# eragonruan/text-detection-ctpn

Measured on NVIDIA H100. Metric: images/sec @600x900, higher is better.
Workload: dtype fp32-faithful: fp16 operands + e4m3 cross terms (1 fp16 + 1 e4m3 wgmma per 16 MACs: 2 bf16-rate units per MAC), fp32 accumulate; matmuls around the BiLSTM on bf16x2

## Files before the change

text-detection-ctpn_b200/csrc/conv_tc.cu:

```cuda
#include <cuda.h>

#include <algorithm>
#include <mutex>
#include <unordered_map>

#include "common.cuh"
#include "tc_ptx.cuh"
#include "tma_host.cuh"

namespace ctpn {

#ifdef CTPN_DEBUG
#define CTPN_DBG(p, bit) (((p).debug & (bit)) != 0)
#else
#define CTPN_DBG(p, bit) false
#endif

struct ConvTcParams {
  int B, H, W, Cin, Cout, taps, planes, flags;
  int tiles_x, tiles_y, tiles_n, total_tiles;
  int m_tiles, total_units;
  int TH, TW, tw_log2;
  int PW;
  int patch_bytes;
  int patch_tx_bytes;
  int group_stride_bytes;
  int cout_pad;
  int Ho, Wo;
  int stages_a, stages_b;
  int debug;
  const float *bias;
  void *out;
  long long out_plane_stride;
  float inv_main, inv_cross, out_s, out_t, out_rs;
  int in_stack_h, out_rows, out_stacked;
  const int *ext;
  int ext_shift, ext_n;
  double work;
  int promote_every;
};

template <int BN, int PR> constexpr bool kEpiWarpgroup = !PR && BN <= 128;
template <int BN, int PR> constexpr int kTcThreads = kEpiWarpgroup<BN, PR> ? 512 : 384;
constexpr int kMaxStages = 8;
constexpr int kCtrlBytes = 8 * (4 * kMaxStages) + 16;
constexpr int kEpiBytes = 2 * 128 * 32 * 4;
constexpr int kXposeBytes = 4 * 512;

struct EpiPixel {
  bool ok, live;
  int oy, ox;
  long long pix;
  unsigned okmask;
  long long spix[4];
};

__device__ __forceinline__ void epi_pixel(const ConvTcParams &p, int mt, int m, int lane, EpiPixel &e) {
  const int th = m >> p.tw_log2, tw = m & (p.TW - 1);
  const int tiles_per_img = p.tiles_x * p.tiles_y;
  const int b = mt / tiles_per_img, r = mt % tiles_per_img;
  const int y = (r / p.tiles_x) * p.TH + th, x = (r % p.tiles_x) * p.TW + tw;
  e.live = true;
  int ob = b;
  if (p.flags & CTPN_F_POOL) {
    e.oy = y >> 1; e.ox = x >> 1;
    e.ok = !(th & 1) && !(tw & 1) && e.oy < p.Ho && e.ox < p.Wo;
  } else {
    e.oy = y; e.ox = x;
    e.ok = y < p.H && x < p.W;
    if (p.in_stack_h) {
      ob = y / p.in_stack_h;
      e.oy = y - ob * p.in_stack_h;
      e.live = e.oy < p.in_stack_h - 1;
      if (!p.out_stacked) e.ok = e.ok && e.live;
    }
  }
  if (p.ext) {
    const int ib = min(ob, p.ext_n - 1);
    e.live = e.live && e.oy < (__ldg(p.ext + 2 * ib) >> p.ext_shift) && e.ox < (__ldg(p.ext + 2 * ib + 1) >> p.ext_shift);
  }
  e.pix = ((long long)ob * p.out_rows + e.oy) * p.Wo + e.ox;
  e.okmask = __ballot_sync(0xffffffffu, e.ok);
#pragma unroll
  for (int it = 0; it < 4; ++it) {
    const long long hi = __shfl_sync(0xffffffffu, (int)(e.pix >> 32), it * 8 + (lane >> 2));
    const unsigned lo = __shfl_sync(0xffffffffu, (unsigned)(e.pix & 0xffffffffll), it * 8 + (lane >> 2));
    e.spix[it] = (hi << 32) | lo;
  }
}

__device__ __forceinline__ void store_transposed(uint4 *stage_w, const uint32_t (&w)[16], uint8_t *obase, long long row_bytes,
                                                 const EpiPixel &e, bool st_ok, bool small, int lane) {
  const int j = lane & 3;
  if (!small) {
    __syncwarp();
#pragma unroll
    for (int q = 0; q < 4; ++q) stage_w[lane * 4 + (q ^ ((lane >> 1) & 3))] = make_uint4(w[4 * q], w[4 * q + 1], w[4 * q + 2], w[4 * q + 3]);
    __syncwarp();
    if (st_ok) {
#pragma unroll
      for (int it = 0; it < 4; ++it) {
        const int pp = it * 8 + (lane >> 2);
        const uint4 val = stage_w[pp * 4 + (j ^ ((pp >> 1) & 3))];
        if ((e.okmask >> pp) & 1u) *reinterpret_cast<uint4 *>(obase + e.spix[it] * row_bytes) = val;
      }
    }
  } else {
#pragma unroll
    for (int it = 0; it < 4; ++it) {
      __syncwarp();
      if ((lane >> 3) == it) {
        const int row = lane & 7;
#pragma unroll
        for (int q = 0; q < 4; ++q) stage_w[row * 4 + (q ^ ((row >> 1) & 3))] = make_uint4(w[4 * q], w[4 * q + 1], w[4 * q + 2], w[4 * q + 3]);
      }
      __syncwarp();
      const int row = lane >> 2, pp = it * 8 + row;
      const uint4 val = stage_w[row * 4 + (j ^ ((row >> 1) & 3))];
      if (st_ok && ((e.okmask >> pp) & 1u)) *reinterpret_cast<uint4 *>(obase + e.spix[it] * row_bytes) = val;
    }
  }
}

template <int P, int F8>
__device__ __forceinline__ void epi_chunk(const ConvTcParams &p, const EpiPixel &e, float (&v)[32], int c0, uint4 *stage_w,
                                          bool small, bool bias_relu, int lane) {
  const bool pool = (p.flags & CTPN_F_POOL) != 0, relu = (p.flags & CTPN_F_RELU) != 0;
  const bool out_f32 = (p.flags & CTPN_F_OUT_F32) != 0;
  if (bias_relu) {
#pragma unroll
    for (int q = 0; q < 8; ++q) {
      const float4 bq = __ldg(reinterpret_cast<const float4 *>(p.bias + c0) + q);
      v[4 * q + 0] += bq.x;
      v[4 * q + 1] += bq.y;
      v[4 * q + 2] += bq.z;
      v[4 * q + 3] += bq.w;
    }
    if (relu) {
#pragma unroll
      for (int i = 0; i < 32; ++i) v[i] = fmaxf(v[i], 0.f);
    }
  }
  if (!e.live) {
#pragma unroll
    for (int i = 0; i < 32; ++i) v[i] = 0.f;
  }
  if (pool) {
#pragma unroll
    for (int i = 0; i < 32; ++i) {
      v[i] = fmaxf(v[i], __shfl_xor_sync(0xffffffffu, v[i], 1));
      v[i] = fmaxf(v[i], __shfl_xor_sync(0xffffffffu, v[i], p.TW));
    }
  }
  if (F8 && pool && !out_f32 && !(p.flags & CTPN_F_OUT_BF16X2)) {
    const int j = (lane & 1) | ((lane >> 2) & 2);
    float x[8];
#pragma unroll
    for (int k = 0; k < 8; ++k) x[k] = j == 0 ? v[k] : j == 1 ? v[8 + k] : j == 2 ? v[16 + k] : v[24 + k];
    const bool okw = e.oy < p.Ho && e.ox < p.Wo;
    uint4 hw;
    uint2 qv, qr;
    f16f8_quad(x[0], x[1], x[2], x[3], p.out_s, p.out_t, p.out_rs, hw.x, hw.y, qv.x, qr.x);
    f16f8_quad(x[4], x[5], x[6], x[7], p.out_s, p.out_t, p.out_rs, hw.z, hw.w, qv.y, qr.y);
    if (okw && c0 < p.Cout && !CTPN_DBG(p, 8)) {
      uint8_t *o0 = reinterpret_cast<uint8_t *>(p.out) + e.pix * p.Cout * 2;
      uint8_t *o1 = o0 + p.out_plane_stride * 2 + (long long)(c0 >> 6) * 128 + (c0 & 63) + j * 8;
      *reinterpret_cast<uint4 *>(o0 + (long long)c0 * 2 + j * 16) = hw;
      *reinterpret_cast<uint2 *>(o1) = qv;
      *reinterpret_cast<uint2 *>(o1 + 64) = qr;
    }
  } else if (F8 && !out_f32 && !(p.flags & CTPN_F_OUT_BF16X2)) {
    uint32_t wh[16], wq[16];
#pragma unroll
    for (int i = 0; i < 8; ++i) {
      f16f8_quad(v[4 * i], v[4 * i + 1], v[4 * i + 2], v[4 * i + 3], p.out_s, p.out_t, p.out_rs, wh[2 * i], wh[2 * i + 1], wq[i], wq[8 + i]);
    }
    const int j = lane & 3;
    const bool st_ok = c0 < p.Cout && !CTPN_DBG(p, 8);
    uint8_t *obase = reinterpret_cast<uint8_t *>(p.out);
    store_transposed(stage_w, wh, obase + (long long)c0 * 2 + j * 16, (long long)p.Cout * 2, e, st_ok, small, lane);
    store_transposed(stage_w, wq, obase + p.out_plane_stride * 2 + (long long)(c0 >> 6) * 128 + (c0 & 63) + (j >> 1) * 64 + (j & 1) * 16,
                     (long long)p.Cout * 2, e, st_ok, small, lane);
  } else if (!out_f32) {
    uint32_t w[P][16];
#pragma unroll
    for (int i = 0; i < 16; ++i) {
      uint32_t t[P];
      split_planes2<P>(v[2 * i], v[2 * i + 1], t);
#pragma unroll
      for (int pl = 0; pl < P; ++pl) w[pl][i] = t[pl];
    }
#pragma unroll
    for (int pl = 0; pl < P; ++pl) {
      uint8_t *obase = reinterpret_cast<uint8_t *>(reinterpret_cast<__nv_bfloat16 *>(p.out) + (long long)pl * p.out_plane_stride + c0 + (lane & 3) * 8);
      store_transposed(stage_w, w[pl], obase, (long long)p.Cout * 2, e, c0 < p.Cout && !CTPN_DBG(p, 8), small, lane);
    }
  } else if (e.ok && c0 < p.Cout && !CTPN_DBG(p, 8)) {
    float4 *dst = reinterpret_cast<float4 *>(reinterpret_cast<float *>(p.out) + e.pix * p.Cout + c0);
#pragma unroll
    for (int q = 0; q < 8; ++q) dst[q] = make_float4(v[4 * q], v[4 * q + 1], v[4 * q + 2], v[4 * q + 3]);
  }
}

template <int BN, int P, int TAPS, int MC, int F8, int PR = 0>
__global__ void __launch_bounds__(kTcThreads<BN, PR>, 1)
conv_tc_kernel(const __grid_constant__ CUtensorMap tmap_a, const __grid_constant__ CUtensorMap tmap_b,
               const ConvTcParams p) {
  using namespace ptx;
  constexpr int kBBytes = BN * 128;
  constexpr bool EW = kEpiWarpgroup<BN, PR>;
  static_assert(!F8 || P == 2, "F16F8 uses two stage slots per operand");
  static_assert(!PR || (P == 3 && !F8), "promotion is built for three bf16 planes");
  extern __shared__ uint8_t smem_raw[];
  const uint32_t raw = smem_u32(smem_raw);
  const uint32_t ring_a = (raw + 1023u) & ~1023u;
  const uint32_t a_stage = (uint32_t)P * p.patch_bytes, b_stage = (uint32_t)P * kBBytes;
  const uint32_t ring_b = ring_a + (uint32_t)p.stages_a * a_stage;
  float *epi = reinterpret_cast<float *>(smem_raw + (ring_b - raw) + (size_t)p.stages_b * b_stage);
  uint4 *xpose = reinterpret_cast<uint4 *>(reinterpret_cast<uint8_t *>(epi) + kEpiBytes);
  uint8_t *ctrl = reinterpret_cast<uint8_t *>(epi) + kEpiBytes + (EW ? kXposeBytes : 0);
  const uint32_t fullA = smem_u32(ctrl), emptyA = fullA + 8 * kMaxStages;
  const uint32_t fullB = emptyA + 8 * kMaxStages, emptyB = fullB + 8 * kMaxStages;
  const uint32_t epiF = emptyB + 8 * kMaxStages, epiE = epiF + 8;

  const int warp = __shfl_sync(0xffffffffu, (int)(threadIdx.x >> 5), 0), lane = threadIdx.x & 31;
  if (threadIdx.x == 0) {
    prefetch_tmap(&tmap_a);
    prefetch_tmap(&tmap_b);
    for (int s = 0; s < kMaxStages; ++s) {
      mbar_init(fullA + 8 * s, 1);
      mbar_init(emptyA + 8 * s, 2);
      mbar_init(fullB + 8 * s, 1);
      mbar_init(emptyB + 8 * s, MC ? 4 : 2);
    }
    mbar_init(epiF, 256);
    mbar_init(epiE, 128);
    fence_mbar_init();
  }
  __syncthreads();
  if (MC) cluster_sync_all();
  const uint32_t rank = MC ? cluster_ctarank() : 0u;
  const int u_begin = MC ? (int)(blockIdx.x >> 1) : (int)blockIdx.x, u_step = MC ? (int)(gridDim.x >> 1) : (int)gridDim.x;
  auto unit_tile = [&](int u, int &mt, int &nt) {
    nt = u % p.tiles_n;
    mt = u / p.tiles_n;
    if (MC) mt = min(2 * mt + (int)rank, p.m_tiles - 1);
  };

  const int kblocks = p.Cin / 64;
  const int tiles_per_img = p.tiles_x * p.tiles_y;
  constexpr int halo = TAPS == 9 ? 1 : 0;

  if (warp < 4) {
    if (EW) regs_dealloc<24>();
    else regs_dealloc<40>();
    if (warp == 1) {
      int s = 0;
      uint32_t ph = 0;
      for (int u = u_begin; u < p.total_units; u += u_step) {
        int mt, nt;
        unit_tile(u, mt, nt);
        const int b = mt / tiles_per_img, r = mt % tiles_per_img;
        const int y0 = (r / p.tiles_x) * p.TH - halo, x0 = (r % p.tiles_x) * p.TW - halo;
        for (int kb = 0; kb < kblocks; ++kb) {
          mbar_wait(emptyA + 8 * s, ph ^ 1u);
          if (elect_one()) {
            if (CTPN_DBG(p, 2)) { mbar_arrive(fullA + 8 * s); }
            else {
              mbar_arrive_expect_tx(fullA + 8 * s, (uint32_t)P * (uint32_t)p.patch_tx_bytes);
              for (int pl = 0; pl < P; ++pl)
                tma_load_4d(&tmap_a, fullA + 8 * s, ring_a + s * a_stage + pl * p.patch_bytes, kb * 64, x0, y0, pl * p.B + b);
            }
          }
          __syncwarp();
          if (++s == p.stages_a) { s = 0; ph ^= 1u; }
        }
      }
    } else if (warp == 0) {
      int s = 0;
      uint32_t ph = 0;
      for (int u = u_begin; u < p.total_units; u += u_step) {
        int mt, nt;
        unit_tile(u, mt, nt);
        for (int kb = 0; kb < kblocks; ++kb) {
          for (int tap = 0; tap < TAPS; ++tap) {
            mbar_wait(emptyB + 8 * s, ph ^ 1u);
            if (elect_one()) {
              if (CTPN_DBG(p, 1)) { mbar_arrive(fullB + 8 * s); }
              else {
                mbar_arrive_expect_tx(fullB + 8 * s, b_stage);
                for (int pl = 0; pl < P; ++pl) {
                  if (MC)
                    tma_load_2d_mc(&tmap_b, fullB + 8 * s, ring_b + s * b_stage + pl * kBBytes + rank * (kBBytes / 2),
                                   tap * p.Cin + kb * 64, pl * p.cout_pad + nt * BN + (int)rank * (BN / 2), (uint16_t)3);
                  else
                    tma_load_2d(&tmap_b, fullB + 8 * s, ring_b + s * b_stage + pl * kBBytes, tap * p.Cin + kb * 64,
                                pl * p.cout_pad + nt * BN);
                }
              }
            }
            __syncwarp();
            if (++s == p.stages_b) { s = 0; ph ^= 1u; }
          }
        }
      }
    }
  } else if (EW && warp >= 12) {
    regs_alloc<152>();
    const int m = (warp & 3) * 32 + lane;
    uint4 *stage_w = xpose + (warp & 3) * 32;
    uint32_t eph = 0;
    if (!CTPN_DBG(p, 16)) {
      for (int u = u_begin; u < p.total_units; u += u_step) {
        int mt, nt;
        unit_tile(u, mt, nt);
        EpiPixel e;
        epi_pixel(p, mt, m, lane, e);
#pragma unroll 1
        for (int c2 = 0; c2 < BN / 64; ++c2) {
          float v[2][32];
          mbar_wait(epiF, eph);
#pragma unroll
          for (int es = 0; es < 2; ++es) {
#pragma unroll
            for (int q = 0; q < 8; ++q) {
              const float4 t = *reinterpret_cast<const float4 *>(epi + es * 4096 + m * 32 + ((q ^ (m & 7)) << 2));
              v[es][4 * q + 0] = t.x; v[es][4 * q + 1] = t.y; v[es][4 * q + 2] = t.z; v[es][4 * q + 3] = t.w;
            }
          }
          mbar_arrive(epiE);
          eph ^= 1u;
#pragma unroll
          for (int es = 0; es < 2; ++es) epi_chunk<P, F8>(p, e, v[es], nt * BN + (2 * c2 + es) * 32, stage_w, true, false, lane);
        }
      }
    }
  } else {
    if (EW) regs_alloc<168>();
    else regs_alloc<232>();
    const int wg = (warp >> 2) - 1;
    const bool leader = (threadIdx.x & 127) == 0;
    constexpr int R = BN / 2;
    float accm[R], accc[R];
    float accs[R];
#ifdef CTPN_DEBUG
    const int pe = PR ? p.promote_every : 1;
#else
    constexpr int pe = 1;
#endif
    constexpr uint32_t kPatch16 = (TAPS == 9 ? 23552u : 16384u) >> 4;
    constexpr uint32_t kB16 = (uint32_t)kBBytes >> 4;
    constexpr uint32_t kHiB = gmma_desc_hi(1024);
    const uint32_t hi_a = gmma_desc_hi((uint32_t)p.group_stride_bytes);
    const uint32_t wg_off = (uint32_t)wg * 8u * (uint32_t)p.group_stride_bytes;
    int sa = 0, sb = 0, prev_b = -1, prev_a = -1;
    uint32_t pha = 0, phb = 0, eph = 0;
    const int frow = wg * 64 + (warp & 3) * 16 + (lane >> 2);
    auto stage_half = [&](int c2) {
#pragma unroll
      for (int j = 0; j < 8; ++j) {
        const int i8 = c2 * 8 + j, q = 2 * (j & 3) + ((lane & 3) >> 1);
#pragma unroll
        for (int h = 0; h < 2; ++h) {
          const int row = frow + 8 * h;
          *reinterpret_cast<float2 *>(epi + (j >> 2) * 4096 + row * 32 + ((q ^ (row & 7)) << 2) + 2 * (lane & 1)) =
              make_float2(accm[4 * i8 + 2 * h], accm[4 * i8 + 2 * h + 1]);
        }
      }
    };
    auto release = [&](int sbx, int sax) {
      if (leader) {
        if (MC) {
          mbar_arrive_cluster(emptyB + 8 * sbx, 0u);
          mbar_arrive_cluster(emptyB + 8 * sbx, 1u);
        } else {
          mbar_arrive(emptyB + 8 * sbx);
        }
        if (sax >= 0) mbar_arrive(emptyA + 8 * sax);
      }
    };
    for (int u = u_begin; u < p.total_units; u += u_step) {
      if (PR) {
#pragma unroll
        for (int i = 0; i < R; ++i) accs[i] = 0.f;
      }
      for (int kb = 0; kb < kblocks; ++kb) {
        if (p.stages_a == 1 && prev_a >= 0) {
          wgmma_wait<0>();
          release(prev_b, prev_a);
          prev_b = prev_a = -1;
        }
        mbar_wait(fullA + 8 * sa, pha);
        const uint32_t a_lo = gmma_desc_lo(ring_a + sa * a_stage + wg_off);
#pragma unroll
        for (int tap = 0; tap < TAPS; ++tap) {
          mbar_wait(fullB + 8 * sb, phb);
          const uint32_t b_lo = gmma_desc_lo(ring_b + sb * b_stage);
          constexpr int kPW = 10;
          const uint32_t view16 = TAPS == 9 ? (uint32_t)((tap / 3) * kPW + tap % 3) * 8u : 0u;
          const uint32_t not_first = (kb | tap) != 0;
          const int step = kb * TAPS + tap;
          wgmma_fence();
          if (!CTPN_DBG(p, 4)) {
            if (F8) {
#pragma unroll
              for (int k = 0; k < 4; ++k)
                wgmma_f16(accm, ((uint64_t)hi_a << 32) | (a_lo + view16 + 2u * k), ((uint64_t)kHiB << 32) | (b_lo + 2u * k),
                          k == 0 ? not_first : 1u);
#pragma unroll
              for (int k = 0; k < 4; ++k)
                wgmma_e4m3(accc, ((uint64_t)hi_a << 32) | (a_lo + kPatch16 + view16 + 2u * k),
                           ((uint64_t)kHiB << 32) | (b_lo + kB16 + 2u * k), k == 0 ? not_first : 1u);
            } else if (PR) {
              const uint32_t chain_on = step % pe != 0;
#pragma unroll
              for (int k = 0; k < 4; ++k)
                wgmma_bf16(accm, ((uint64_t)hi_a << 32) | (a_lo + view16 + 2u * k), ((uint64_t)kHiB << 32) | (b_lo + 2u * k),
                           k == 0 ? chain_on : 1u);
              wgmma_commit();
#pragma unroll
              for (int i = 0; i < P; ++i) {
#pragma unroll
                for (int j = (i == 0); j < P - i; ++j) {
#pragma unroll
                  for (int k = 0; k < 4; ++k) {
                    const uint64_t da = ((uint64_t)hi_a << 32) | (a_lo + i * kPatch16 + view16 + 2u * k);
                    const uint64_t db = ((uint64_t)kHiB << 32) | (b_lo + j * kB16 + 2u * k);
                    wgmma_bf16(accc, da, db, (k == 0 && i == 0 && j == 1) ? not_first : 1u);
                  }
                }
              }
            } else {
#pragma unroll
              for (int i = 0; i < P; ++i) {
#pragma unroll
                for (int j = 0; j < P - i; ++j) {
#pragma unroll
                  for (int k = 0; k < 4; ++k) {
                    const uint64_t da = ((uint64_t)hi_a << 32) | (a_lo + i * kPatch16 + view16 + 2u * k);
                    const uint64_t db = ((uint64_t)kHiB << 32) | (b_lo + j * kB16 + 2u * k);
                    if (i + j == 0) wgmma_bf16(accm, da, db, k == 0 ? not_first : 1u);
                    else wgmma_bf16(accc, da, db, (k == 0 && i == 0 && j == 1) ? not_first : 1u);
                  }
                }
              }
            }
          }
          wgmma_commit();
          wgmma_wait<1>();
          if (prev_b >= 0) release(prev_b, prev_a);
          prev_b = sb;
          prev_a = tap == TAPS - 1 ? sa : -1;
          if (PR && ((step + 1) % pe == 0 || step == kblocks * TAPS - 1)) {
            wgmma_fence_regs(accm);
#pragma unroll
            for (int i = 0; i < R; ++i) accs[i] = __fadd_rn(accs[i], accm[i]);
          }
          if (++sb == p.stages_b) { sb = 0; phb ^= 1u; }
        }
        if (++sa == p.stages_a) { sa = 0; pha ^= 1u; }
      }
      wgmma_wait<0>();
      wgmma_fence_regs(accm);
      if (P > 1) wgmma_fence_regs(accc);
      if (prev_b >= 0) release(prev_b, prev_a);
      prev_b = prev_a = -1;
      if (P > 1) {
#pragma unroll
        for (int i = 0; i < R; ++i)
          accm[i] = F8 ? __fmaf_rn(accc[i], p.inv_cross, accm[i] * p.inv_main) : PR ? __fadd_rn(accs[i], accc[i]) : accm[i] + accc[i];
      }

      if (CTPN_DBG(p, 16)) continue;
      if (EW) {
        const float *bt = p.bias + (u % p.tiles_n) * BN + 2 * (lane & 3);
#pragma unroll
        for (int i8 = 0; i8 < BN / 8; ++i8) {
          const float2 bq = __ldg(reinterpret_cast<const float2 *>(bt + 8 * i8));
#pragma unroll
          for (int h = 0; h < 2; ++h) {
            accm[4 * i8 + 2 * h] += bq.x;
            accm[4 * i8 + 2 * h + 1] += bq.y;
          }
        }
        if (p.flags & CTPN_F_RELU) {
#pragma unroll
          for (int i = 0; i < R; ++i) accm[i] = fmaxf(accm[i], 0.f);
        }
#pragma unroll
        for (int c2 = 0; c2 < BN / 64; ++c2) {
          mbar_wait(epiE, eph ^ 1u);
          stage_half(c2);
          mbar_arrive(epiF);
          eph ^= 1u;
        }
      } else {
        const int cw = warp - 4, eset = cw >> 2, quarter = cw & 3;
        const int m = quarter * 32 + lane;
        int mt, nt;
        unit_tile(u, mt, nt);
        EpiPixel e;
        epi_pixel(p, mt, m, lane, e);
        uint4 *stage_w = reinterpret_cast<uint4 *>(epi + eset * 4096 + quarter * 1024);
#pragma unroll
        for (int c2 = 0; c2 < BN / 64; ++c2) {
          named_sync(1, 256);
          stage_half(c2);
          named_sync(1, 256);
          float v[32];
#pragma unroll
          for (int q = 0; q < 8; ++q) {
            const float4 t = *reinterpret_cast<const float4 *>(epi + eset * 4096 + m * 32 + ((q ^ (m & 7)) << 2));
            v[4 * q + 0] = t.x; v[4 * q + 1] = t.y; v[4 * q + 2] = t.z; v[4 * q + 3] = t.w;
          }
          epi_chunk<P, F8>(p, e, v, nt * BN + (2 * c2 + eset) * 32, stage_w, false, true, lane);
        }
      }
    }
  }
  __syncthreads();
  if (MC) cluster_sync_all();
}


constexpr int kMaxDevices = 64;
static std::mutex g_mu;
static int g_sms[kMaxDevices];

struct Tuning { int debug = 0, bn = 0, stages_a = 0, stages_b = 0, mcast = 1, promote = 1; };
static const Tuning &tuning() {
  static const Tuning t = [] {
    Tuning v;
#ifdef CTPN_DEBUG
    auto env_int = [](const char *name, int dflt) { const char *e = getenv(name); return e ? atoi(e) : dflt; };
    v.debug = env_int("CTPN_TC_DEBUG", 0);
    v.bn = env_int("CTPN_TC_BN", 0);
    v.stages_a = env_int("CTPN_TC_STAGES_A", 0);
    v.stages_b = env_int("CTPN_TC_STAGES_B", 0);
    v.mcast = env_int("CTPN_TC_MCAST", 1);
    v.promote = std::max(1, env_int("CTPN_TC_PROMOTE", 1));
#endif
    return v;
  }();
  return t;
}

struct TmapKey {
  const void *ptr;
  unsigned long long d0, d1, d2, d3;
  unsigned b0, b1, b2, b3;
  int dev;
  bool operator==(const TmapKey &o) const {
    return ptr == o.ptr && d0 == o.d0 && d1 == o.d1 && d2 == o.d2 && d3 == o.d3 && b0 == o.b0 && b1 == o.b1 && b2 == o.b2 &&
           b3 == o.b3 && dev == o.dev;
  }
};
struct TmapKeyHash {
  size_t operator()(const TmapKey &k) const {
    size_t h = std::hash<const void *>()(k.ptr);
    for (unsigned long long v : {k.d0, k.d1, k.d2, k.d3, (unsigned long long)k.b0, (unsigned long long)k.b1,
                                 (unsigned long long)k.b2, (unsigned long long)k.b3, (unsigned long long)k.dev})
      h = h * 1000003u ^ std::hash<unsigned long long>()(v);
    return h;
  }
};
static std::unordered_map<TmapKey, CUtensorMap, TmapKeyHash> g_tmaps;

static int cached_tmap(int dev, CUtensorMap *out, const void *ptr, int rank, const cuuint64_t *dims, const cuuint64_t *strides,
                       const cuuint32_t *box) {
  TmapKey k{ptr, dims[0], dims[1], rank > 2 ? dims[2] : 0, rank > 3 ? dims[3] : 0, box[0], box[1], rank > 2 ? box[2] : 0,
            rank > 3 ? box[3] : 0, dev};
  std::lock_guard<std::mutex> lock(g_mu);
  auto it = g_tmaps.find(k);
  if (it != g_tmaps.end()) { *out = it->second; return CTPN_OK; }
  EncodeTiledFn enc = nullptr;
  int rc = tma_get_encode(&enc);
  if (rc) return rc;
  if ((rc = tma_encode_bf16(enc, out, const_cast<void *>(ptr), rank, dims, strides, box))) return rc;
  if (g_tmaps.size() >= 1024) g_tmaps.clear();
  g_tmaps.emplace(k, *out);
  return CTPN_OK;
}

template <int BN, int P, int TAPS, int MC, int F8 = 0, int PR = 0>
static int launch_bn(int dev, const CUtensorMap &ta, const CUtensorMap &tb, ConvTcParams &p, cudaStream_t st) {
  const size_t a_stage = (size_t)p.planes * p.patch_bytes, b_stage = (size_t)p.planes * BN * 128;
  const size_t epi_bytes = kEpiBytes + (kEpiWarpgroup<BN, PR> ? kXposeBytes : 0);
  const size_t budget = 227 * 1024 - 1024 - kCtrlBytes - epi_bytes;
  int sa = (2 * a_stage + 2 * b_stage <= budget) ? 2 : 1;
  if (p.taps == 1) sa = (int)std::min<size_t>(4, std::max<size_t>(1, (budget / 2) / a_stage));
  CTPN_REQUIRE(sa * a_stage + 2 * b_stage <= budget, "conv_tc: pipeline stages (%zu + 2 x %zu B) do not fit in shared memory", a_stage, b_stage);
  int sb = (int)((budget - sa * a_stage) / b_stage);
  if (sb > kMaxStages) sb = kMaxStages;
  if (tuning().stages_a > 0) sa = std::max(1, std::min(sa, tuning().stages_a));
  if (tuning().stages_b > 0) sb = std::max(2, std::min(sb, tuning().stages_b));
  p.stages_a = sa;
  p.stages_b = sb;
  const size_t smem = 1024 + sa * a_stage + sb * b_stage + epi_bytes + kCtrlBytes;
  CTPN_REQUIRE(smem <= 227 * 1024, "conv_tc: %zu bytes of shared memory", smem);
  auto kernel = conv_tc_kernel<BN, P, TAPS, MC, F8, PR>;
  static bool attr_set[kMaxDevices];
  static int max_clusters[kMaxDevices];
  cudaLaunchConfig_t cfg = {};
  cudaLaunchAttribute attr;
  attr.id = cudaLaunchAttributeClusterDimension;
  attr.val.clusterDim.x = 2; attr.val.clusterDim.y = 1; attr.val.clusterDim.z = 1;
  cfg.blockDim = dim3(kTcThreads<BN, PR>);
  cfg.dynamicSmemBytes = smem;
  cfg.stream = st;
  cfg.attrs = &attr;
  cfg.numAttrs = MC ? 1 : 0;
  {
    std::lock_guard<std::mutex> lock(g_mu);
    if (!attr_set[dev]) {
      CTPN_CUDA(cudaFuncSetAttribute(kernel, cudaFuncAttributeMaxDynamicSharedMemorySize, 227 * 1024));
      if (MC) {
        cfg.gridDim = dim3(2 * (g_sms[dev] / 2));
        int n = 0;
        CTPN_CUDA(cudaOccupancyMaxActiveClusters(&n, kernel, &cfg));
        CTPN_REQUIRE(n > 0, "conv_tc: no 2-CTA cluster of this kernel fits on the device");
        max_clusters[dev] = n;
      }
      attr_set[dev] = true;
    }
  }
  char label[128];
  if (prof_enabled()) snprintf(label, sizeof(label), "conv_tc t%d %dx%dx%d c%d-%d %s%d bn%d%s%s", p.taps, p.B, p.H, p.W, p.Cin, p.Cout, F8 ? "f16f8 p" : "p", p.planes, BN, MC ? " mc" : "", PR ? " promote" : "");
  ProfScope prof(label, p.work, st);
  if (MC) cfg.gridDim = dim3(2 * std::min(max_clusters[dev], p.total_units));
  else cfg.gridDim = dim3(std::min(p.total_units, g_sms[dev]));
  CTPN_CUDA(cudaLaunchKernelEx(&cfg, kernel, ta, tb, p));
  CTPN_LAUNCH_CHECK();
  return CTPN_OK;
}

int conv_tc_run(const void *in_planes, const void *w_planes, const float *bias, void *out, int B, int H, int W, int cin,
                int cout, int taps, int planes, int flags, const QuantScales *q, const int *ext, int ext_shift, void *stream) {
  const bool f8 = q != nullptr, promote = (flags & CTPN_F_PROMOTE) != 0;
  CTPN_REQUIRE(f8 || !(flags & CTPN_F_OUT_BF16X2), "ctpn_conv3x3: CTPN_F_OUT_BF16X2 is a flag of ctpn_conv3x3_f16f8");
  CTPN_REQUIRE(!(promote && f8), "ctpn_conv3x3_f16f8: CTPN_F_PROMOTE is a flag of ctpn_conv3x3 with planes = 3");
  CTPN_REQUIRE(!promote || planes == 3, "ctpn_conv3x3: CTPN_F_PROMOTE needs planes = 3 (got %d)", planes);
  CTPN_REQUIRE(in_planes && w_planes && bias && out, "ctpn_conv3x3: null pointer");
  CTPN_REQUIRE(taps == 9 || taps == 1, "ctpn_conv3x3: taps must be 9 or 1 (got %d)", taps);
  CTPN_REQUIRE(planes >= 1 && planes <= 3, "ctpn_conv3x3: planes must be 1..3 (got %d)", planes);
  CTPN_REQUIRE(cin % 64 == 0 && cin >= 64, "ctpn_conv3x3: Cin must be a multiple of 64 (got %d)", cin);
  CTPN_REQUIRE(cout % 64 == 0 && cout >= 64, "ctpn_conv3x3: Cout must be a multiple of 64 (got %d)", cout);
  CTPN_REQUIRE(B > 0 && H > 0 && W > 0, "ctpn_conv3x3: bad shape");
  const bool pool = flags & CTPN_F_POOL;
  CTPN_REQUIRE(!pool || (taps == 9 && H >= 2 && W >= 2), "ctpn_conv3x3: pooling needs taps=9 and H,W >= 2");
  const bool stack_in = flags & CTPN_F_STACK_IN, stack_out = flags & CTPN_F_STACK_OUT;
  CTPN_REQUIRE(!stack_in || (taps == 9 && !pool), "ctpn_conv3x3: CTPN_F_STACK_IN needs taps=9 and no pooling");
  CTPN_REQUIRE(!stack_out || !(flags & CTPN_F_OUT_F32), "ctpn_conv3x3: stacked output is a plane format");
  const int img_B = B, img_H = H;
  if (stack_in) {
    CTPN_REQUIRE((long long)B * (H + 1) < (1ll << 30), "ctpn_conv3x3: stack too tall");
    H = B * (H + 1);
    B = 1;
  }
  int dev = 0, rc;
  CTPN_CUDA(cudaGetDevice(&dev));
  CTPN_REQUIRE(dev >= 0 && dev < kMaxDevices, "ctpn_conv3x3: device index %d not supported", dev);
  {
    std::lock_guard<std::mutex> lock(g_mu);
    if (g_sms[dev] == 0) CTPN_CUDA(cudaDeviceGetAttribute(&g_sms[dev], cudaDevAttrMultiProcessorCount, dev));
  }

  ConvTcParams p;
  memset(&p, 0, sizeof(p));
  p.B = B; p.H = H; p.W = W; p.Cin = cin; p.Cout = cout; p.taps = taps; p.planes = planes; p.flags = flags;
  if (taps == 9) {
    p.TH = 16; p.TW = 8; p.tw_log2 = 3;
    p.PW = 10;
    p.group_stride_bytes = p.PW * 128;
    p.patch_tx_bytes = p.PW * 18 * 128;
    p.patch_bytes = (int)align_up((size_t)p.patch_tx_bytes, 1024);
  } else {
    p.TH = 1; p.TW = 128; p.tw_log2 = 7;
    p.PW = 128;
    p.group_stride_bytes = 1024;
    p.patch_tx_bytes = 128 * 128;
    p.patch_bytes = 128 * 128;
  }
  p.tiles_x = ceil_div(W, p.TW);
  p.tiles_y = ceil_div(H, p.TH);
  p.Ho = pool ? H / 2 : H;
  p.Wo = pool ? W / 2 : W;
  p.bias = bias;
  p.out = out;
  p.work = 2.0 * img_B * img_H * W * (double)taps * cin * cout;
  p.in_stack_h = stack_in ? img_H + 1 : 0;
  const int img_Ho = pool ? img_H / 2 : img_H;
  p.out_rows = img_Ho + (stack_out ? 1 : 0);
  p.out_stacked = stack_out ? 1 : 0;
  p.out_plane_stride = (long long)img_B * p.out_rows * p.Wo * cout;
  p.cout_pad = cout;
  p.ext = ext;
  p.ext_shift = ext_shift;
  p.ext_n = img_B;
  if (f8) {
    CTPN_REQUIRE(q->inv_main > 0.f && q->inv_cross > 0.f && q->out_s > 0.f && q->out_t > 0.f, "ctpn_conv3x3_f16f8: scales must be positive");
    p.inv_main = q->inv_main; p.inv_cross = q->inv_cross; p.out_s = q->out_s; p.out_t = q->out_t;
    p.out_rs = kResidualGain * q->out_t / q->out_s;
  }
  p.debug = tuning().debug;
  p.promote_every = tuning().promote;

  int BN = tuning().bn > 0 ? tuning().bn : (planes == 1 ? 256 : 128);
  if (!(BN == 64 || BN == 128 || BN == 256)) BN = 256;
  if (planes > 1 && BN > 128) BN = 128;
  while (BN > cout || cout % BN) BN >>= 1;
  const long long m_tiles = (long long)B * p.tiles_x * p.tiles_y;
  constexpr long long kMcMaxTilesPerSm = 16;
  const bool mc = taps == 9 && tuning().mcast != 0 && m_tiles >= 2 &&
                  (promote || m_tiles * (cout / BN) < kMcMaxTilesPerSm * g_sms[dev]);
  if (promote && taps == 9 && !mc && BN > 64) BN = 64;
  p.tiles_n = cout / BN;
  const long long total = m_tiles * p.tiles_n;
  CTPN_REQUIRE(total < (1ll << 31), "ctpn_conv3x3: too many tiles");
  p.total_tiles = (int)total;
  p.m_tiles = (int)m_tiles;
  p.total_units = mc ? (int)((m_tiles + 1) / 2) * p.tiles_n : p.total_tiles;

  CUtensorMap ta, tb;
  {
    const int halo = taps == 9 ? 1 : 0;
    cuuint64_t dims[4] = {(cuuint64_t)cin, (cuuint64_t)W, (cuuint64_t)H, (cuuint64_t)planes * B};
    cuuint64_t strides[3] = {(cuuint64_t)cin * 2, (cuuint64_t)W * cin * 2, (cuuint64_t)H * W * cin * 2};
    cuuint32_t box[4] = {64, (cuuint32_t)p.PW, (cuuint32_t)(p.TH + 2 * halo), 1};
    if ((rc = cached_tmap(dev, &ta, in_planes, 4, dims, strides, box))) return rc;
  }
  {
    cuuint64_t dims[2] = {(cuuint64_t)taps * cin, (cuuint64_t)planes * cout};
    cuuint64_t strides[1] = {(cuuint64_t)taps * cin * 2};
    cuuint32_t box[2] = {64, (cuuint32_t)(mc ? BN / 2 : BN)};
    if ((rc = cached_tmap(dev, &tb, w_planes, 2, dims, strides, box))) return rc;
  }
  cudaStream_t st = (cudaStream_t)stream;
#define CTPN_TC_CASE(BN_, P_, T_) \
  if (BN == BN_ && planes == P_ && taps == T_) return launch_bn<BN_, P_, T_, 0>(dev, ta, tb, p, st)
#define CTPN_TC_CASE_MC(BN_, P_) \
  if (mc && BN == BN_ && planes == P_) return launch_bn<BN_, P_, 9, 1>(dev, ta, tb, p, st)
  if (f8) {
    if (mc && BN == 128) return launch_bn<128, 2, 9, 1, 1>(dev, ta, tb, p, st);
    if (mc && BN == 64) return launch_bn<64, 2, 9, 1, 1>(dev, ta, tb, p, st);
    if (taps == 9 && BN == 128) return launch_bn<128, 2, 9, 0, 1>(dev, ta, tb, p, st);
    if (taps == 9 && BN == 64) return launch_bn<64, 2, 9, 0, 1>(dev, ta, tb, p, st);
    if (taps == 1 && BN == 128) return launch_bn<128, 2, 1, 0, 1>(dev, ta, tb, p, st);
    if (taps == 1 && BN == 64) return launch_bn<64, 2, 1, 0, 1>(dev, ta, tb, p, st);
    set_error("ctpn_conv3x3_f16f8: no kernel for BN=%d taps=%d", BN, taps);
    return CTPN_ERR_INVALID;
  }
  if (promote) {
    if (mc && BN == 128) return launch_bn<128, 3, 9, 1, 0, 1>(dev, ta, tb, p, st);
    if (mc && BN == 64) return launch_bn<64, 3, 9, 1, 0, 1>(dev, ta, tb, p, st);
    if (taps == 9 && BN == 64) return launch_bn<64, 3, 9, 0, 0, 1>(dev, ta, tb, p, st);
    if (taps == 1 && BN == 128) return launch_bn<128, 3, 1, 0, 0, 1>(dev, ta, tb, p, st);
    if (taps == 1 && BN == 64) return launch_bn<64, 3, 1, 0, 0, 1>(dev, ta, tb, p, st);
    set_error("ctpn_conv3x3: no promoted kernel for BN=%d taps=%d", BN, taps);
    return CTPN_ERR_INVALID;
  }
  CTPN_TC_CASE_MC(256, 1); CTPN_TC_CASE_MC(128, 1); CTPN_TC_CASE_MC(64, 1);
  CTPN_TC_CASE_MC(128, 2); CTPN_TC_CASE_MC(64, 2);
  CTPN_TC_CASE_MC(128, 3); CTPN_TC_CASE_MC(64, 3);
  CTPN_TC_CASE(256, 1, 9); CTPN_TC_CASE(128, 1, 9); CTPN_TC_CASE(64, 1, 9);
  CTPN_TC_CASE(128, 2, 9); CTPN_TC_CASE(64, 2, 9);
  CTPN_TC_CASE(128, 3, 9); CTPN_TC_CASE(64, 3, 9);
  CTPN_TC_CASE(256, 1, 1); CTPN_TC_CASE(128, 1, 1); CTPN_TC_CASE(64, 1, 1);
  CTPN_TC_CASE(128, 2, 1); CTPN_TC_CASE(64, 2, 1);
  CTPN_TC_CASE(128, 3, 1); CTPN_TC_CASE(64, 3, 1);
#undef CTPN_TC_CASE_MC
#undef CTPN_TC_CASE
  set_error("ctpn_conv3x3: no kernel for BN=%d planes=%d taps=%d", BN, planes, taps);
  return CTPN_ERR_INVALID;
}

}

using namespace ctpn;

extern "C" int ctpn_conv3x3(const void *in_planes, const void *w_planes, const float *bias, void *out, int B, int H,
                            int W, int cin, int cout, int taps, int planes, int flags, void *stream) {
  return conv_tc_run(in_planes, w_planes, bias, out, B, H, W, cin, cout, taps, planes, flags, nullptr, nullptr, 0, stream);
}

extern "C" int ctpn_conv3x3_f16f8(const void *in_planes, const void *w_planes, const float *bias, void *out, int B, int H,
                                  int W, int cin, int cout, int taps, int flags, float inv_main, float inv_cross, float out_s,
                                  float out_t, void *stream) {
  const QuantScales q{inv_main, inv_cross, out_s, out_t};
  return conv_tc_run(in_planes, w_planes, bias, out, B, H, W, cin, cout, taps, 2, flags, &q, nullptr, 0, stream);
}
```

Measured before the change: 817.7.

## Restructure conv epilogue with double-buffered staging, in-register pooling, and direct stores

```diff
diff --git a/text-detection-ctpn_b200/csrc/conv_tc.cu b/text-detection-ctpn_b200/csrc/conv_tc.cu
--- a/text-detection-ctpn_b200/csrc/conv_tc.cu
+++ b/text-detection-ctpn_b200/csrc/conv_tc.cu
@@ -43,162 +43,88 @@
 template <int BN, int PR> constexpr bool kEpiWarpgroup = !PR && BN <= 128;
 template <int BN, int PR> constexpr int kTcThreads = kEpiWarpgroup<BN, PR> ? 512 : 384;
 constexpr int kMaxStages = 8;
-constexpr int kCtrlBytes = 8 * (4 * kMaxStages) + 16;
-constexpr int kEpiBytes = 2 * 128 * 32 * 4;
-constexpr int kXposeBytes = 4 * 512;
+constexpr int kCtrlBytes = 8 * (4 * kMaxStages) + 32;
+constexpr int kEpiSlotFloats = 128 * 32;
+constexpr int kEpiBytes = 2 * kEpiSlotFloats * 4;
+
+__device__ __forceinline__ int stage_chunk(int q, int row) { return q ^ (row & 7) ^ ((q >> 3) & 1); }
+
+__device__ __forceinline__ void load_piece(const float *stage, int rw, int row, int j, float (&x)[8]) {
+  const float *r = stage + row * rw;
+  const float4 a = *reinterpret_cast<const float4 *>(r + (stage_chunk(2 * j, row) << 2));
+  const float4 b = *reinterpret_cast<const float4 *>(r + (stage_chunk(2 * j + 1, row) << 2));
+  x[0] = a.x; x[1] = a.y; x[2] = a.z; x[3] = a.w; x[4] = b.x; x[5] = b.y; x[6] = b.z; x[7] = b.w;
+}
 
 struct EpiPixel {
-  bool ok, live;
-  int oy, ox;
   long long pix;
-  unsigned okmask;
-  long long spix[4];
+  bool live;
 };
 
-__device__ __forceinline__ void epi_pixel(const ConvTcParams &p, int mt, int m, int lane, EpiPixel &e) {
-  const int th = m >> p.tw_log2, tw = m & (p.TW - 1);
+__device__ __forceinline__ EpiPixel epi_pixel(const ConvTcParams &p, int mt, int row) {
+  const bool pool = (p.flags & CTPN_F_POOL) != 0;
+  const int half = p.TW >> 1;
+  const int th = pool ? (row / half) * 2 : row >> p.tw_log2, tw = pool ? (row % half) * 2 : row & (p.TW - 1);
   const int tiles_per_img = p.tiles_x * p.tiles_y;
   const int b = mt / tiles_per_img, r = mt % tiles_per_img;
   const int y = (r / p.tiles_x) * p.TH + th, x = (r % p.tiles_x) * p.TW + tw;
-  e.live = true;
-  int ob = b;
-  if (p.flags & CTPN_F_POOL) {
-    e.oy = y >> 1; e.ox = x >> 1;
-    e.ok = !(th & 1) && !(tw & 1) && e.oy < p.Ho && e.ox < p.Wo;
+  bool live = true, ok;
+  int ob = b, oy, ox;
+  if (pool) {
+    oy = y >> 1; ox = x >> 1;
+    ok = oy < p.Ho && ox < p.Wo;
   } else {
-    e.oy = y; e.ox = x;
-    e.ok = y < p.H && x < p.W;
+    oy = y; ox = x;
+    ok = y < p.H && x < p.W;
     if (p.in_stack_h) {
       ob = y / p.in_stack_h;
-      e.oy = y - ob * p.in_stack_h;
-      e.live = e.oy < p.in_stack_h - 1;
-      if (!p.out_stacked) e.ok = e.ok && e.live;
+      oy = y - ob * p.in_stack_h;
+      live = oy < p.in_stack_h - 1;
+      if (!p.out_stacked) ok = ok && live;
     }
   }
   if (p.ext) {
     const int ib = min(ob, p.ext_n - 1);
-    e.live = e.live && e.oy < (__ldg(p.ext + 2 * ib) >> p.ext_shift) && e.ox < (__ldg(p.ext + 2 * ib + 1) >> p.ext_shift);
-  }
-  e.pix = ((long long)ob * p.out_rows + e.oy) * p.Wo + e.ox;
-  e.okmask = __ballot_sync(0xffffffffu, e.ok);
-#pragma unroll
-  for (int it = 0; it < 4; ++it) {
-    const long long hi = __shfl_sync(0xffffffffu, (int)(e.pix >> 32), it * 8 + (lane >> 2));
-    const unsigned lo = __shfl_sync(0xffffffffu, (unsigned)(e.pix & 0xffffffffll), it * 8 + (lane >> 2));
-    e.spix[it] = (hi << 32) | lo;
-  }
-}
-
-__device__ __forceinline__ void store_transposed(uint4 *stage_w, const uint32_t (&w)[16], uint8_t *obase, long long row_bytes,
-                                                 const EpiPixel &e, bool st_ok, bool small, int lane) {
-  const int j = lane & 3;
-  if (!small) {
-    __syncwarp();
-#pragma unroll
-    for (int q = 0; q < 4; ++q) stage_w[lane * 4 + (q ^ ((lane >> 1) & 3))] = make_uint4(w[4 * q], w[4 * q + 1], w[4 * q + 2], w[4 * q + 3]);
-    __syncwarp();
-    if (st_ok) {
-#pragma unroll
-      for (int it = 0; it < 4; ++it) {
-        const int pp = it * 8 + (lane >> 2);
-        const uint4 val = stage_w[pp * 4 + (j ^ ((pp >> 1) & 3))];
-        if ((e.okmask >> pp) & 1u) *reinterpret_cast<uint4 *>(obase + e.spix[it] * row_bytes) = val;
-      }
-    }
-  } else {
-#pragma unroll
-    for (int it = 0; it < 4; ++it) {
-      __syncwarp();
-      if ((lane >> 3) == it) {
-        const int row = lane & 7;
-#pragma unroll
-        for (int q = 0; q < 4; ++q) stage_w[row * 4 + (q ^ ((row >> 1) & 3))] = make_uint4(w[4 * q], w[4 * q + 1], w[4 * q + 2], w[4 * q + 3]);
-      }
-      __syncwarp();
-      const int row = lane >> 2, pp = it * 8 + row;
-      const uint4 val = stage_w[row * 4 + (j ^ ((row >> 1) & 3))];
-      if (st_ok && ((e.okmask >> pp) & 1u)) *reinterpret_cast<uint4 *>(obase + e.spix[it] * row_bytes) = val;
-    }
-  }
+    live = live && oy < (__ldg(p.ext + 2 * ib) >> p.ext_shift) && ox < (__ldg(p.ext + 2 * ib + 1) >> p.ext_shift);
+  }
+  return EpiPixel{ok ? ((long long)ob * p.out_rows + oy) * p.Wo + ox : -1ll, live};
 }
 
 template <int P, int F8>
-__device__ __forceinline__ void epi_chunk(const ConvTcParams &p, const EpiPixel &e, float (&v)[32], int c0, uint4 *stage_w,
-                                          bool small, bool bias_relu, int lane) {
-  const bool pool = (p.flags & CTPN_F_POOL) != 0, relu = (p.flags & CTPN_F_RELU) != 0;
-  const bool out_f32 = (p.flags & CTPN_F_OUT_F32) != 0;
-  if (bias_relu) {
-#pragma unroll
-    for (int q = 0; q < 8; ++q) {
-      const float4 bq = __ldg(reinterpret_cast<const float4 *>(p.bias + c0) + q);
-      v[4 * q + 0] += bq.x;
-      v[4 * q + 1] += bq.y;
-      v[4 * q + 2] += bq.z;
-      v[4 * q + 3] += bq.w;
-    }
-    if (relu) {
-#pragma unroll
-      for (int i = 0; i < 32; ++i) v[i] = fmaxf(v[i], 0.f);
-    }
-  }
+__device__ __forceinline__ void store_piece(const ConvTcParams &p, const EpiPixel &e, int c, float (&x)[8]) {
+  if (e.pix < 0 || CTPN_DBG(p, 8)) return;
   if (!e.live) {
 #pragma unroll
-    for (int i = 0; i < 32; ++i) v[i] = 0.f;
-  }
-  if (pool) {
-#pragma unroll
-    for (int i = 0; i < 32; ++i) {
-      v[i] = fmaxf(v[i], __shfl_xor_sync(0xffffffffu, v[i], 1));
-      v[i] = fmaxf(v[i], __shfl_xor_sync(0xffffffffu, v[i], p.TW));
-    }
-  }
-  if (F8 && pool && !out_f32 && !(p.flags & CTPN_F_OUT_BF16X2)) {
-    const int j = (lane & 1) | ((lane >> 2) & 2);
-    float x[8];
-#pragma unroll
-    for (int k = 0; k < 8; ++k) x[k] = j == 0 ? v[k] : j == 1 ? v[8 + k] : j == 2 ? v[16 + k] : v[24 + k];
-    const bool okw = e.oy < p.Ho && e.ox < p.Wo;
+    for (int i = 0; i < 8; ++i) x[i] = 0.f;
+  }
+  uint8_t *o = reinterpret_cast<uint8_t *>(p.out);
+  if (p.flags & CTPN_F_OUT_F32) {
+    float4 *dst = reinterpret_cast<float4 *>(reinterpret_cast<float *>(p.out) + e.pix * p.Cout + c);
+    dst[0] = make_float4(x[0], x[1], x[2], x[3]);
+    dst[1] = make_float4(x[4], x[5], x[6], x[7]);
+  } else if (F8 && !(p.flags & CTPN_F_OUT_BF16X2)) {
     uint4 hw;
     uint2 qv, qr;
     f16f8_quad(x[0], x[1], x[2], x[3], p.out_s, p.out_t, p.out_rs, hw.x, hw.y, qv.x, qr.x);
     f16f8_quad(x[4], x[5], x[6], x[7], p.out_s, p.out_t, p.out_rs, hw.z, hw.w, qv.y, qr.y);
-    if (okw && c0 < p.Cout && !CTPN_DBG(p, 8)) {
-      uint8_t *o0 = reinterpret_cast<uint8_t *>(p.out) + e.pix * p.Cout * 2;
-      uint8_t *o1 = o0 + p.out_plane_stride * 2 + (long long)(c0 >> 6) * 128 + (c0 & 63) + j * 8;
-      *reinterpret_cast<uint4 *>(o0 + (long long)c0 * 2 + j * 16) = hw;
-      *reinterpret_cast<uint2 *>(o1) = qv;
-      *reinterpret_cast<uint2 *>(o1 + 64) = qr;
-    }
-  } else if (F8 && !out_f32 && !(p.flags & CTPN_F_OUT_BF16X2)) {
-    uint32_t wh[16], wq[16];
-#pragma unroll
-    for (int i = 0; i < 8; ++i) {
-      f16f8_quad(v[4 * i], v[4 * i + 1], v[4 * i + 2], v[4 * i + 3], p.out_s, p.out_t, p.out_rs, wh[2 * i], wh[2 * i + 1], wq[i], wq[8 + i]);
-    }
-    const int j = lane & 3;
-    const bool st_ok = c0 < p.Cout && !CTPN_DBG(p, 8);
-    uint8_t *obase = reinterpret_cast<uint8_t *>(p.out);
-    store_transposed(stage_w, wh, obase + (long long)c0 * 2 + j * 16, (long long)p.Cout * 2, e, st_ok, small, lane);
-    store_transposed(stage_w, wq, obase + p.out_plane_stride * 2 + (long long)(c0 >> 6) * 128 + (c0 & 63) + (j >> 1) * 64 + (j & 1) * 16,
-                     (long long)p.Cout * 2, e, st_ok, small, lane);
-  } else if (!out_f32) {
-    uint32_t w[P][16];
-#pragma unroll
-    for (int i = 0; i < 16; ++i) {
+    uint8_t *o0 = o + e.pix * p.Cout * 2;
+    uint8_t *o1 = o0 + p.out_plane_stride * 2 + (c >> 6) * 128 + (c & 63);
+    *reinterpret_cast<uint4 *>(o0 + c * 2) = hw;
+    *reinterpret_cast<uint2 *>(o1) = qv;
+    *reinterpret_cast<uint2 *>(o1 + 64) = qr;
+  } else {
+    uint32_t w[P][4];
+#pragma unroll
+    for (int i = 0; i < 4; ++i) {
       uint32_t t[P];
-      split_planes2<P>(v[2 * i], v[2 * i + 1], t);
+      split_planes2<P>(x[2 * i], x[2 * i + 1], t);
 #pragma unroll
       for (int pl = 0; pl < P; ++pl) w[pl][i] = t[pl];
     }
 #pragma unroll
-    for (int pl = 0; pl < P; ++pl) {
-      uint8_t *obase = reinterpret_cast<uint8_t *>(reinterpret_cast<__nv_bfloat16 *>(p.out) + (long long)pl * p.out_plane_stride + c0 + (lane & 3) * 8);
-      store_transposed(stage_w, w[pl], obase, (long long)p.Cout * 2, e, c0 < p.Cout && !CTPN_DBG(p, 8), small, lane);
-    }
-  } else if (e.ok && c0 < p.Cout && !CTPN_DBG(p, 8)) {
-    float4 *dst = reinterpret_cast<float4 *>(reinterpret_cast<float *>(p.out) + e.pix * p.Cout + c0);
-#pragma unroll
-    for (int q = 0; q < 8; ++q) dst[q] = make_float4(v[4 * q], v[4 * q + 1], v[4 * q + 2], v[4 * q + 3]);
+    for (int pl = 0; pl < P; ++pl)
+      *reinterpret_cast<uint4 *>(o + ((long long)pl * p.out_plane_stride + e.pix * p.Cout + c) * 2) =
+          make_uint4(w[pl][0], w[pl][1], w[pl][2], w[pl][3]);
   }
 }
 
@@ -217,11 +143,11 @@
   const uint32_t a_stage = (uint32_t)P * p.patch_bytes, b_stage = (uint32_t)P * kBBytes;
   const uint32_t ring_b = ring_a + (uint32_t)p.stages_a * a_stage;
   float *epi = reinterpret_cast<float *>(smem_raw + (ring_b - raw) + (size_t)p.stages_b * b_stage);
-  uint4 *xpose = reinterpret_cast<uint4 *>(reinterpret_cast<uint8_t *>(epi) + kEpiBytes);
-  uint8_t *ctrl = reinterpret_cast<uint8_t *>(epi) + kEpiBytes + (EW ? kXposeBytes : 0);
+  uint8_t *ctrl = reinterpret_cast<uint8_t *>(epi) + kEpiBytes;
   const uint32_t fullA = smem_u32(ctrl), emptyA = fullA + 8 * kMaxStages;
   const uint32_t fullB = emptyA + 8 * kMaxStages, emptyB = fullB + 8 * kMaxStages;
-  const uint32_t epiF = emptyB + 8 * kMaxStages, epiE = epiF + 8;
+  const uint32_t epiF = emptyB + 8 * kMaxStages, epiE = epiF + 16;
+  const bool pool = (p.flags & CTPN_F_POOL) != 0;
 
   const int warp = __shfl_sync(0xffffffffu, (int)(threadIdx.x >> 5), 0), lane = threadIdx.x & 31;
   if (threadIdx.x == 0) {
@@ -233,8 +159,10 @@
       mbar_init(fullB + 8 * s, 1);
       mbar_init(emptyB + 8 * s, MC ? 4 : 2);
     }
-    mbar_init(epiF, 256);
-    mbar_init(epiE, 128);
+    for (int s = 0; s < 2; ++s) {
+      mbar_init(epiF + 8 * s, 256);
+      mbar_init(epiE + 8 * s, 128);
+    }
     fence_mbar_init();
   }
   __syncthreads();
@@ -307,31 +235,55 @@
     }
   } else if (EW && warp >= 12) {
     regs_alloc<152>();
-    const int m = (warp & 3) * 32 + lane;
-    uint4 *stage_w = xpose + (warp & 3) * 32;
+    const int t = threadIdx.x & 127, j = t & 7;
     uint32_t eph = 0;
+    int slot = 0;
     if (!CTPN_DBG(p, 16)) {
       for (int u = u_begin; u < p.total_units; u += u_step) {
         int mt, nt;
         unit_tile(u, mt, nt);
-        EpiPixel e;
-        epi_pixel(p, mt, m, lane, e);
+        if (pool) {
+          constexpr int NB = BN / 64;
+          EpiPixel e[2];
+          float v[2][NB][8];
+#pragma unroll
+          for (int k = 0; k < 2; ++k) e[k] = epi_pixel(p, mt, (t >> 3) + 16 * k);
+          mbar_wait(epiF + 8 * slot, (eph >> slot) & 1u);
+          const float *src = epi + slot * kEpiSlotFloats;
+#pragma unroll
+          for (int k = 0; k < 2; ++k)
+#pragma unroll
+            for (int c2 = 0; c2 < NB; ++c2) load_piece(src, BN, (t >> 3) + 16 * k, j + 8 * c2, v[k][c2]);
+          mbar_arrive(epiE + 8 * slot);
+          eph ^= 1u << slot;
+          slot ^= 1;
+#pragma unroll
+          for (int k = 0; k < 2; ++k)
+#pragma unroll
+            for (int c2 = 0; c2 < NB; ++c2) store_piece<P, F8>(p, e[k], nt * BN + 64 * c2 + 8 * j, v[k][c2]);
+        } else {
+          const int j4 = t & 3;
+          EpiPixel e[4];
+#pragma unroll
+          for (int k = 0; k < 4; ++k) e[k] = epi_pixel(p, mt, (t >> 2) + 32 * k);
+          constexpr int QL = P == 3 ? 1 : 2;
 #pragma unroll 1
-        for (int c2 = 0; c2 < BN / 64; ++c2) {
-          float v[2][32];
-          mbar_wait(epiF, eph);
-#pragma unroll
-          for (int es = 0; es < 2; ++es) {
-#pragma unroll
-            for (int q = 0; q < 8; ++q) {
-              const float4 t = *reinterpret_cast<const float4 *>(epi + es * 4096 + m * 32 + ((q ^ (m & 7)) << 2));
-              v[es][4 * q + 0] = t.x; v[es][4 * q + 1] = t.y; v[es][4 * q + 2] = t.z; v[es][4 * q + 3] = t.w;
+          for (int c = 0; c < BN / 32; c += QL) {
+            float v[QL][4][8];
+#pragma unroll
+            for (int hq = 0; hq < QL; ++hq) {
+              mbar_wait(epiF + 8 * slot, (eph >> slot) & 1u);
+#pragma unroll
+              for (int k = 0; k < 4; ++k) load_piece(epi + slot * kEpiSlotFloats, 32, (t >> 2) + 32 * k, j4, v[hq][k]);
+              mbar_arrive(epiE + 8 * slot);
+              eph ^= 1u << slot;
+              slot ^= 1;
             }
+#pragma unroll
+            for (int hq = 0; hq < QL; ++hq)
+#pragma unroll
+              for (int k = 0; k < 4; ++k) store_piece<P, F8>(p, e[k], nt * BN + 32 * (c + hq) + 8 * j4, v[hq][k]);
           }
-          mbar_arrive(epiE);
-          eph ^= 1u;
-#pragma unroll
-          for (int es = 0; es < 2; ++es) epi_chunk<P, F8>(p, e, v[es], nt * BN + (2 * c2 + es) * 32, stage_w, true, false, lane);
         }
       }
     }
@@ -355,17 +307,36 @@
     const uint32_t wg_off = (uint32_t)wg * 8u * (uint32_t)p.group_stride_bytes;
     int sa = 0, sb = 0, prev_b = -1, prev_a = -1;
     uint32_t pha = 0, phb = 0, eph = 0;
+    int eslot = 0;
     const int frow = wg * 64 + (warp & 3) * 16 + (lane >> 2);
-    auto stage_half = [&](int c2) {
-#pragma unroll
-      for (int j = 0; j < 8; ++j) {
-        const int i8 = c2 * 8 + j, q = 2 * (j & 3) + ((lane & 3) >> 1);
+    auto stage_quarter = [&](float *dst, int c4) {
+#pragma unroll
+      for (int j = 0; j < 4; ++j) {
+        const int i8 = c4 * 4 + j, q = 2 * j + ((lane & 3) >> 1);
 #pragma unroll
         for (int h = 0; h < 2; ++h) {
           const int row = frow + 8 * h;
-          *reinterpret_cast<float2 *>(epi + (j >> 2) * 4096 + row * 32 + ((q ^ (row & 7)) << 2) + 2 * (lane & 1)) =
+          *reinterpret_cast<float2 *>(dst + row * 32 + (stage_chunk(q, row) << 2) + 2 * (lane & 1)) =
               make_float2(accm[4 * i8 + 2 * h], accm[4 * i8 + 2 * h + 1]);
         }
+      }
+    };
+    auto stage_pooled = [&](float *dst) {
+      const int b = (lane >> 2) & 1;
+      const int row = (wg * 4 + (warp & 3)) * 4 + (lane >> 3);
+#pragma unroll
+      for (int x = 0; x < BN / 8; ++x) {
+        if (x & 2) continue;
+        float r[2];
+#pragma unroll
+        for (int k = 0; k < 2; ++k) {
+          const float lo = fmaxf(accm[4 * x + k], accm[4 * x + 2 + k]);
+          const float hi = fmaxf(accm[4 * (x + 2) + k], accm[4 * (x + 2) + 2 + k]);
+          const float recv = __shfl_xor_sync(0xffffffffu, b ? lo : hi, 4);
+          r[k] = fmaxf(b ? hi : lo, recv);
+        }
+        const int q = 2 * (x | (b << 1)) + ((lane & 3) >> 1);
+        *reinterpret_cast<float2 *>(dst + row * BN + (stage_chunk(q, row) << 2) + 2 * (lane & 1)) = make_float2(r[0], r[1]);
       }
     };
     auto release = [&](int sbx, int sax) {
@@ -472,48 +443,72 @@
       }
 
       if (CTPN_DBG(p, 16)) continue;
+      const float *bt = p.bias + (u % p.tiles_n) * BN + 2 * (lane & 3);
+#pragma unroll
+      for (int i8 = 0; i8 < BN / 8; ++i8) {
+        const float2 bq = __ldg(reinterpret_cast<const float2 *>(bt + 8 * i8));
+#pragma unroll
+        for (int h = 0; h < 2; ++h) {
+          accm[4 * i8 + 2 * h] += bq.x;
+          accm[4 * i8 + 2 * h + 1] += bq.y;
+        }
+      }
+      if (p.flags & CTPN_F_RELU) {
+#pragma unroll
+        for (int i = 0; i < R; ++i) accm[i] = fmaxf(accm[i], 0.f);
+      }
       if (EW) {
-        const float *bt = p.bias + (u % p.tiles_n) * BN + 2 * (lane & 3);
-#pragma unroll
-        for (int i8 = 0; i8 < BN / 8; ++i8) {
-          const float2 bq = __ldg(reinterpret_cast<const float2 *>(bt + 8 * i8));
-#pragma unroll
-          for (int h = 0; h < 2; ++h) {
-            accm[4 * i8 + 2 * h] += bq.x;
-            accm[4 * i8 + 2 * h + 1] += bq.y;
+        if (pool) {
+          mbar_wait(epiE + 8 * eslot, ((eph >> eslot) & 1u) ^ 1u);
+          stage_pooled(epi + eslot * kEpiSlotFloats);
+          mbar_arrive(epiF + 8 * eslot);
+          eph ^= 1u << eslot;
+          eslot ^= 1;
+        } else {
+#pragma unroll
+          for (int c4 = 0; c4 < BN / 32; ++c4) {
+            const int s = c4 & 1;
+            mbar_wait(epiE + 8 * s, ((eph >> s) & 1u) ^ 1u);
+            stage_quarter(epi + s * kEpiSlotFloats, c4);
+            mbar_arrive(epiF + 8 * s);
+            eph ^= 1u << s;
           }
         }
-        if (p.flags & CTPN_F_RELU) {
-#pragma unroll
-          for (int i = 0; i < R; ++i) accm[i] = fmaxf(accm[i], 0.f);
-        }
-#pragma unroll
-        for (int c2 = 0; c2 < BN / 64; ++c2) {
-          mbar_wait(epiE, eph ^ 1u);
-          stage_half(c2);
-          mbar_arrive(epiF);
-          eph ^= 1u;
-        }
       } else {
-        const int cw = warp - 4, eset = cw >> 2, quarter = cw & 3;
-        const int m = quarter * 32 + lane;
+        const int t = threadIdx.x - 128, j = t & 7;
         int mt, nt;
         unit_tile(u, mt, nt);
-        EpiPixel e;
-        epi_pixel(p, mt, m, lane, e);
-        uint4 *stage_w = reinterpret_cast<uint4 *>(epi + eset * 4096 + quarter * 1024);
-#pragma unroll
-        for (int c2 = 0; c2 < BN / 64; ++c2) {
+        if (pool) {
+          const EpiPixel e = epi_pixel(p, mt, t >> 3);
           named_sync(1, 256);
-          stage_half(c2);
+          stage_pooled(epi);
           named_sync(1, 256);
-          float v[32];
-#pragma unroll
-          for (int q = 0; q < 8; ++q) {
-            const float4 t = *reinterpret_cast<const float4 *>(epi + eset * 4096 + m * 32 + ((q ^ (m & 7)) << 2));
-            v[4 * q + 0] = t.x; v[4 * q + 1] = t.y; v[4 * q + 2] = t.z; v[4 * q + 3] = t.w;
+#pragma unroll
+          for (int c2 = 0; c2 < BN / 64; ++c2) {
+            float v[8];
+            load_piece(epi, BN, t >> 3, j + 8 * c2, v);
+            store_piece<P, F8>(p, e, nt * BN + 64 * c2 + 8 * j, v);
           }
-          epi_chunk<P, F8>(p, e, v, nt * BN + (2 * c2 + eset) * 32, stage_w, false, true, lane);
+        } else {
+          const int j4 = t & 3;
+          EpiPixel e[2];
+#pragma unroll
+          for (int k = 0; k < 2; ++k) e[k] = epi_pixel(p, mt, (t >> 2) + 64 * k);
+#pragma unroll
+          for (int c2 = 0; c2 < BN / 64; ++c2) {
+            named_sync(1, 256);
+            stage_quarter(epi, 2 * c2);
+            stage_quarter(epi + kEpiSlotFloats, 2 * c2 + 1);
+            named_sync(1, 256);
+#pragma unroll
+            for (int hq = 0; hq < 2; ++hq)
+#pragma unroll
+              for (int k = 0; k < 2; ++k) {
+                float v[8];
+                load_piece(epi + hq * kEpiSlotFloats, 32, (t >> 2) + 64 * k, j4, v);
+                store_piece<P, F8>(p, e[k], nt * BN + 64 * c2 + 32 * hq + 8 * j4, v);
+              }
+          }
         }
       }
     }
@@ -585,8 +580,7 @@
 template <int BN, int P, int TAPS, int MC, int F8 = 0, int PR = 0>
 static int launch_bn(int dev, const CUtensorMap &ta, const CUtensorMap &tb, ConvTcParams &p, cudaStream_t st) {
   const size_t a_stage = (size_t)p.planes * p.patch_bytes, b_stage = (size_t)p.planes * BN * 128;
-  const size_t epi_bytes = kEpiBytes + (kEpiWarpgroup<BN, PR> ? kXposeBytes : 0);
-  const size_t budget = 227 * 1024 - 1024 - kCtrlBytes - epi_bytes;
+  const size_t budget = 227 * 1024 - 1024 - kCtrlBytes - kEpiBytes;
   int sa = (2 * a_stage + 2 * b_stage <= budget) ? 2 : 1;
   if (p.taps == 1) sa = (int)std::min<size_t>(4, std::max<size_t>(1, (budget / 2) / a_stage));
   CTPN_REQUIRE(sa * a_stage + 2 * b_stage <= budget, "conv_tc: pipeline stages (%zu + 2 x %zu B) do not fit in shared memory", a_stage, b_stage);
@@ -596,7 +590,7 @@
   if (tuning().stages_b > 0) sb = std::max(2, std::min(sb, tuning().stages_b));
   p.stages_a = sa;
   p.stages_b = sb;
-  const size_t smem = 1024 + sa * a_stage + sb * b_stage + epi_bytes + kCtrlBytes;
+  const size_t smem = 1024 + sa * a_stage + sb * b_stage + kEpiBytes + kCtrlBytes;
   CTPN_REQUIRE(smem <= 227 * 1024, "conv_tc: %zu bytes of shared memory", smem);
   auto kernel = conv_tc_kernel<BN, P, TAPS, MC, F8, PR>;
   static bool attr_set[kMaxDevices];
```

Measured after the change: 847.4 (median of 6 runs). +3.6%, better.
